# IN2-ViAUn/Exploration-of-Potential

Hardware: AMD Instinct MI355X
Metric: training images/sec, YOLOX-l 24p 640x640 bf16 (higher is better)
Workload: dtype bf16; 1 GPU; YOLOX-l-24p (CSPDarknet53+PAFPN+24p head) train step, 640x640, batch 20/GPU, 10 GTs/img, SimOTA + 24-circle GIoU loss, SGD nesterov; global_batch=20, parallelism=dp1, hip_graph=forward and backward as two lanes of captured segments, loss, update

## Files before the change

exploration-of-potential_amd/csrc/elementwise.hip:

```cpp
#include <stdio.h>
#include <stdlib.h>
#include "common.h"

namespace {

constexpr int MAX_BLOCKS = 2048;

__device__ __forceinline__ void load8(const bf16* p, float (&v)[8]) {
    bf16x8 t = *reinterpret_cast<const bf16x8*>(p);
#pragma unroll
    for (int i = 0; i < 8; ++i) v[i] = (float)t[i];
}
__device__ __forceinline__ void store8(bf16* p, const float (&v)[8]) {
    bf16x8 t;
#pragma unroll
    for (int i = 0; i < 8; ++i) t[i] = (bf16)v[i];
    *reinterpret_cast<bf16x8*>(p) = t;
}

struct RowMap {
    int tpr, rpb;
    __device__ RowMap(int C, int nt = 256) { tpr = C >> 3; rpb = tpr >= nt ? 1 : nt / tpr; }
};

template <int ACT, bool RES>
__global__ __launch_bounds__(256) void bn_act_fwd_kernel(const bf16* z, long ld_z, const long long* stats, int reps,
                                                         const float* gamma, const float* beta, float* rmean,
                                                         float* rvar, long* nbt, long* nbt2, float* save, bf16* y, long ld_y,
                                                         const bf16* res_, long ld_res, long M, int C, float eps,
                                                         float momentum) {
    constexpr int act = ACT;
    const bf16* res = RES ? res_ : nullptr;
    extern __shared__ float lds[];
    const int CP = C + (C >> 3);
    float* sc = lds;
    float* sh = lds + CP;
    auto pad = [](int c) { return c + (c >> 3); };
    for (int c = threadIdx.x; c < C; c += 256) {
        long long i1 = 0, i2 = 0;
        const float gmm = gamma[c], bta = beta[c];
        for (int rb = 0; rb < reps; rb += 8) {
            long long a[8], b[8];
#pragma unroll
            for (int r = 0; r < 8; ++r) {
                const int rr = rb + r < reps ? rb + r : rb;
                a[r] = stats[(long)rr * 2 * C + c];
                b[r] = stats[(long)rr * 2 * C + C + c];
            }
#pragma unroll
            for (int r = 0; r < 8; ++r) {
                i1 += rb + r < reps ? a[r] : 0ll;
                i2 += rb + r < reps ? b[r] : 0ll;
            }
        }
// ... 582 lines not shown
#pragma unroll
                for (int j = 0; j < 8; ++j) {
                    const unsigned byte = ((j < 4 ? c.x : c.y) >> (8 * (j & 3))) & 0xFFu;
                    if ((int)(byte >> 4) == dy + 8) { s[j] += (float)t[j]; sel[j] = (unsigned char)(byte & 15u); }
                }
            }
#pragma unroll
            for (int j = 0; j < 8; ++j) gh[q * 8 + j] = s[j];
            uint2 d;
            d.x = sel[0] | (sel[1] << 8) | (sel[2] << 16) | ((unsigned)sel[3] << 24);
            d.y = sel[4] | (sel[5] << 8) | (sel[6] << 16) | ((unsigned)sel[7] << 24);
            ds[q] = d;
        }
        __syncthreads();
#pragma unroll
        for (int t = 0; t < NPASS; ++t) {
            const int q = threadIdx.x + 256 * t;
            if (q < HW) {
                const int r = q / W, c = q - r * W;
                for (int dxo = -R; dxo <= R; ++dxo) {
                    const int x = c - dxo;
                    if (x < 0 || x >= W) continue;
                    const int o = r * W + x;
                    const uint2 d = ds[o];
#pragma unroll
                    for (int j = 0; j < 8; ++j) {
                        const unsigned byte = ((j < 4 ? d.x : d.y) >> (8 * (j & 3))) & 0xFFu;
                        if ((int)byte == dxo + 8) acc[t][j] += gh[o * 8 + j];
                    }
                }
            }
        }
        __syncthreads();
    }
#pragma unroll
    for (int t = 0; t < NPASS; ++t) {
        const int q = threadIdx.x + 256 * t;
        if (q < HW) {
            bf16* d = dx + (base + q) * ld_dx + cg * 8;
            float out[8];
#pragma unroll
            for (int j = 0; j < 8; ++j) out[j] = acc[t][j];
            if (accumulate) {
                float o[8];
                load8(d, o);
#pragma unroll
                for (int j = 0; j < 8; ++j) out[j] += o[j];
            }
            store8(d, out);
        }
    }
}

__global__ __launch_bounds__(256) void upsample2_fwd_kernel(const bf16* x, long ld_x, bf16* y, long ld_y, int B, int H,
                                                            int W, int C) {
    const int cgs = C >> 3;
    const long total = (long)B * 2 * H * 2 * W * cgs;
    for (long i = (long)blockIdx.x * 256 + threadIdx.x; i < total; i += (long)gridDim.x * 256) {
        const int cg = (int)(i % cgs);
        const long opix = i / cgs;
        const int n = (int)(opix / (4 * H * W));
        const int rem = (int)(opix - (long)n * 4 * H * W);
        const int oy = rem / (2 * W), ox = rem - oy * 2 * W;
        const long ip = (long)(n * H + (oy >> 1)) * W + (ox >> 1);
        *reinterpret_cast<bf16x8*>(y + opix * ld_y + cg * 8) = *reinterpret_cast<const bf16x8*>(x + ip * ld_x + cg * 8);
    }
}

__global__ __launch_bounds__(256) void upsample2_bwd_kernel(const bf16* dy, long ld_dy, bf16* dx, long ld_dx,
                                                            int accumulate, int B, int H, int W, int C) {
    const int cgs = C >> 3;
    const long total = (long)B * H * W * cgs;
    for (long i = (long)blockIdx.x * 256 + threadIdx.x; i < total; i += (long)gridDim.x * 256) {
        const int cg = (int)(i % cgs);
        const long pix = i / cgs;
        const int n = (int)(pix / (H * W));
        const int rem = (int)(pix - (long)n * H * W);
        const int py = rem / W, px = rem - py * W;
        float acc[8] = {0, 0, 0, 0, 0, 0, 0, 0};
#pragma unroll
        for (int a = 0; a < 2; ++a)
#pragma unroll
            for (int b = 0; b < 2; ++b) {
                float v[8];
                load8(dy + ((long)(n * 2 * H + 2 * py + a) * 2 * W + 2 * px + b) * ld_dy + cg * 8, v);
#pragma unroll
                for (int j = 0; j < 8; ++j) acc[j] += v[j];
            }
        bf16* d = dx + pix * ld_dx + cg * 8;
        if (accumulate) {
            float o[8];
            load8(d, o);
#pragma unroll
            for (int j = 0; j < 8; ++j) acc[j] += o[j];
        }
        store8(d, acc);
    }
}

__global__ __launch_bounds__(256) void rows_copy_kernel(const bf16* src, long ld_src, bf16* dst, long ld_dst,
                                                        int accumulate, long M, int C) {
    const int cgs = C >> 3;
    const long total = M * cgs;
    for (long i = (long)blockIdx.x * 256 + threadIdx.x; i < total; i += (long)gridDim.x * 256) {
        const int cg = (int)(i % cgs);
        const long m = i / cgs;
// ... 393 lines not shown
    EP24_REQUIRE(C % 8 == 0 && C <= 2048 && ld_dy % 8 == 0 && ld_z % 8 == 0 && ld_dz % 8 == 0, EP24_E_ARG, "bn_act_bwd_fused: alignment / C <= 2048");
    EP24_REQUIRE((((uintptr_t)save | (uintptr_t)gamma | (uintptr_t)beta | (uintptr_t)gamma_grad | (uintptr_t)beta_grad) & 15) == 0, EP24_E_ARG,
                 "bn_act_bwd_fused: save / gamma / beta and their gradients must be 16-byte aligned (they are read as vectors)");
    int grid = rows_grid(M, C, 4, 256, 256);
    auto kfn = act == 1 ? bn_act_bwd_fused_kernel<1> : act == 2 ? bn_act_bwd_fused_kernel<2> : act == 3 ? bn_act_bwd_fused_kernel<3> : bn_act_bwd_fused_kernel<0>;
    hipLaunchKernelGGL(kfn, dim3(grid), dim3(256), 2 * (size_t)C * sizeof(float), S_, (const bf16*)dy, ld_dy, (const bf16*)z, ld_z, save, gamma, beta,
                       (long long*)dgamma, (long long*)dbeta, gamma_grad, beta_grad, (bf16*)dz, ld_dz, M, C, reps, (unsigned*)barrier);
    EP24_LAUNCH_CHECK("ep24_bn_act_bwd_fused");
    return EP24_OK;
}

namespace ep24_igemm {
int bn_barrier_timeouts() {
    unsigned v = 0;
    if (hipMemcpyFromSymbol(&v, HIP_SYMBOL(g_bn_barrier_timeouts), sizeof(v)) != hipSuccess) return -1;
    return (int)v;
}
}

extern "C" int ep24_bn_act_bwd_apply_acc(const void* dy, int64_t ld_dy, const void* z, int64_t ld_z, const float* save,
                                         const float* gamma, const float* beta, const int64_t* dgamma, const int64_t* dbeta,
                                         float* gamma_grad, float* beta_grad, void* dz, int64_t ld_dz, int64_t M, int C, int act,
                                         int reps, void* stream) {
    EP24_REQUIRE(dy && z && save && gamma && beta && dgamma && dbeta && dz && reps > 0, EP24_E_ARG, "bn_act_bwd_apply_acc: null pointer / reps");
    EP24_REQUIRE(C % 8 == 0 && ld_dy % 8 == 0 && ld_z % 8 == 0 && ld_dz % 8 == 0, EP24_E_ARG, "bn_act_bwd_apply_acc: alignment");
    EP24_REQUIRE((((uintptr_t)save | (uintptr_t)gamma | (uintptr_t)beta) & 15) == 0, EP24_E_ARG,
                 "bn_act_bwd_apply_acc: save / gamma / beta must be 16-byte aligned (they are read as vectors)");
    EP24_REQUIRE((((uintptr_t)gamma_grad | (uintptr_t)beta_grad) & 15) == 0, EP24_E_ARG, "bn_act_bwd_apply_acc: gamma_grad / beta_grad must be 16-byte aligned");
    auto kfn = act == 1 ? bn_act_bwd_apply_kernel<4, 1, true> : act == 2 ? bn_act_bwd_apply_kernel<4, 2, true> : bn_act_bwd_apply_kernel<4, 0, true>;
    hipLaunchKernelGGL(kfn, dim3(rows_grid(M, C, 16, 2048)), dim3(256), 2 * (size_t)C * sizeof(float), S_, (const bf16*)dy, ld_dy, (const bf16*)z, ld_z, save, gamma, beta,
                       (const long long*)dgamma, (const long long*)dbeta, gamma_grad, beta_grad, (bf16*)dz, ld_dz, M, C, reps);
    EP24_LAUNCH_CHECK("ep24_bn_act_bwd_apply_acc");
    return EP24_OK;
}

extern "C" int ep24_stem_pack(const float* images, void* rows, int64_t ld, int B, int H, int W, void* stream) {
    EP24_REQUIRE(images && rows && H % 2 == 0 && W % 2 == 0 && B > 0 && ld >= 108 && ld % 8 == 0, EP24_E_ARG, "stem_pack: bad arguments");
    long sp_blocks = ((long)B * (H / 2) * (W / 2) + 31) / 32;
    hipLaunchKernelGGL(stem_pack_kernel, dim3((unsigned)(sp_blocks > 16384 ? 16384 : sp_blocks)), dim3(256), 0, S_, images,
                       (bf16*)rows, B, H, W, (int)ld);
    EP24_LAUNCH_CHECK("ep24_stem_pack");
    return EP24_OK;
}

extern "C" int ep24_focus_pack(const float* images, void* f16, int B, int H, int W, void* stream) {
    EP24_REQUIRE(images && f16 && H % 2 == 0 && W % 2 == 0 && B > 0 && (reinterpret_cast<unsigned long long>(images) & 7) == 0, EP24_E_ARG,
                 "focus_pack: bad arguments");
    const long blocks = ((long)B * (H / 2) * (W / 2) + 255) / 256;
    hipLaunchKernelGGL(focus_pack_kernel, dim3((unsigned)(blocks > 65536 ? 65536 : blocks)), dim3(256), 0, S_, images, (bf16*)f16, B, H, W);
    EP24_LAUNCH_CHECK("ep24_focus_pack");
    return EP24_OK;
}

extern "C" int ep24_spp_fwd(const void* x, int64_t ld_x, void* y5, void* y9, void* y13, int64_t ld_y, uint8_t* idx, int B,
                            int H, int W, int C, void* scratch, void* stream) {
    EP24_REQUIRE(x && y5 && y9 && y13 && idx && C % 8 == 0 && ld_x % 8 == 0 && ld_y % 8 == 0, EP24_E_ARG, "spp_fwd: bad arguments");
    if (scratch) {
        const long n = (long)B * H * W * C;
        bf16* h = (bf16*)scratch;
        uint8_t* hx = (uint8_t*)scratch + 6 * n;
        hipLaunchKernelGGL(spp_row_kernel, dim3(cap_grid(n / 8)), dim3(256), 0, S_, (const bf16*)x, ld_x, h, hx, B, H, W, C);
        hipLaunchKernelGGL(spp_col_kernel, dim3(cap_grid(n / 8)), dim3(256), 0, S_, (const bf16*)h, (const uint8_t*)hx, (bf16*)y5,
                           (bf16*)y9, (bf16*)y13, ld_y, idx, B, H, W, C);
        EP24_LAUNCH_CHECK("ep24_spp_fwd");
        return EP24_OK;
    }
    hipLaunchKernelGGL(spp_fwd_kernel, dim3(cap_grid((long)B * H * W * (C / 8))), dim3(256), 0, S_, (const bf16*)x, ld_x,
                       (bf16*)y5, (bf16*)y9, (bf16*)y13, ld_y, idx, B, H, W, C);
    EP24_LAUNCH_CHECK("ep24_spp_fwd");
    return EP24_OK;
}

extern "C" int ep24_spp_bwd(const void* dy5, const void* dy9, const void* dy13, int64_t ld_dy, const uint8_t* idx, void* dx,
                            int64_t ld_dx, int accumulate, int B, int H, int W, int C, void* stream) {
    EP24_REQUIRE(dy5 && dy9 && dy13 && idx && dx && C % 8 == 0 && ld_dy % 8 == 0 && ld_dx % 8 == 0, EP24_E_ARG, "spp_bwd: bad arguments");
    const size_t lds = (size_t)H * W * 112;
    if (lds <= 64 * 1024 && H * W <= 1024)
        hipLaunchKernelGGL(spp_bwd_lds_kernel, dim3(C / 8, B), dim3(256), lds, S_, (const bf16*)dy5, (const bf16*)dy9, (const bf16*)dy13,
                           ld_dy, idx, (bf16*)dx, ld_dx, accumulate, B, H, W, C);
    else
        hipLaunchKernelGGL(spp_bwd_kernel, dim3(cap_grid((long)B * H * W * (C / 8))), dim3(256), 0, S_, (const bf16*)dy5,
                           (const bf16*)dy9, (const bf16*)dy13, ld_dy, idx, (bf16*)dx, ld_dx, accumulate, B, H, W, C);
    EP24_LAUNCH_CHECK("ep24_spp_bwd");
    return EP24_OK;
}

extern "C" int ep24_upsample2_fwd(const void* x, int64_t ld_x, void* y, int64_t ld_y, int B, int H, int W, int C, void* stream) {
    EP24_REQUIRE(x && y && C % 8 == 0 && ld_x % 8 == 0 && ld_y % 8 == 0, EP24_E_ARG, "upsample2_fwd: bad arguments");
    hipLaunchKernelGGL(upsample2_fwd_kernel, dim3(cap_grid((long)B * 4 * H * W * (C / 8))), dim3(256), 0, S_, (const bf16*)x,
                       ld_x, (bf16*)y, ld_y, B, H, W, C);
    EP24_LAUNCH_CHECK("ep24_upsample2_fwd");
    return EP24_OK;
}

extern "C" int ep24_upsample2_bwd(const void* dy, int64_t ld_dy, void* dx, int64_t ld_dx, int accumulate, int B, int H, int W,
                                  int C, void* stream) {
    EP24_REQUIRE(dy && dx && C % 8 == 0 && ld_dy % 8 == 0 && ld_dx % 8 == 0, EP24_E_ARG, "upsample2_bwd: bad arguments");
    hipLaunchKernelGGL(upsample2_bwd_kernel, dim3(cap_grid((long)B * H * W * (C / 8))), dim3(256), 0, S_, (const bf16*)dy, ld_dy,
                       (bf16*)dx, ld_dx, accumulate, B, H, W, C);
    EP24_LAUNCH_CHECK("ep24_upsample2_bwd");
    return EP24_OK;
}

extern "C" int ep24_rows_copy(const void* src, int64_t ld_src, void* dst, int64_t ld_dst, int accumulate, int64_t M, int C,
                              void* stream) {
    EP24_REQUIRE(src && dst && C % 8 == 0 && ld_src % 8 == 0 && ld_dst % 8 == 0, EP24_E_ARG, "rows_copy: bad arguments");
    hipLaunchKernelGGL(rows_copy_kernel, dim3(cap_grid(M * (C / 8))), dim3(256), 0, S_, (const bf16*)src, ld_src, (bf16*)dst,
                       ld_dst, accumulate, M, C);
    EP24_LAUNCH_CHECK("ep24_rows_copy");
    return EP24_OK;
}

extern "C" int ep24_cast_f32_bf16(const float* src, void* dst, int64_t n, void* stream) {
    EP24_REQUIRE(src && dst && n % 4 == 0 && n >= 0, EP24_E_ARG, "cast_f32_bf16: n must be a multiple of 4");
    if (n) hipLaunchKernelGGL(cast_f32_bf16_kernel, dim3(cap_grid(n / 4)), dim3(256), 0, S_, src, (bf16*)dst, (long)(n / 4));
    EP24_LAUNCH_CHECK("ep24_cast_f32_bf16");
    return EP24_OK;
}

extern "C" int ep24_cast_bf16_f32(const void* src, float* dst, int64_t n, void* stream) {
    EP24_REQUIRE(src && dst && n % 4 == 0 && n >= 0, EP24_E_ARG, "cast_bf16_f32: n must be a multiple of 4");
    if (n) hipLaunchKernelGGL(cast_bf16_f32_kernel, dim3(cap_grid(n / 4)), dim3(256), 0, S_, (const bf16*)src, dst, (long)(n / 4));
    EP24_LAUNCH_CHECK("ep24_cast_bf16_f32");
    return EP24_OK;
}

extern "C" int ep24_head_decode_fwd(float* out, int B, int A, int a0, int H, int W, float stride, int ncols, float* origin,
                                    void* stream) {
    EP24_REQUIRE(out && a0 >= 0 && a0 + H * W <= A && ncols >= 27, EP24_E_ARG, "head_decode_fwd: bad arguments");
    hipLaunchKernelGGL(decode_fwd_kernel, dim3(cap_grid((long)B * H * W * 26)), dim3(256), 0, S_, out, B, A, a0, H, W, stride, ncols, origin);
    EP24_LAUNCH_CHECK("ep24_head_decode_fwd");
    return EP24_OK;
}

extern "C" int ep24_head_decode_bwd(const float* dout, const float* out, void* d_regobj, void* d_cls, int B, int A, int a0,
                                    int H, int W, float stride, int ncols, const float* d_origin, void* stream) {
    EP24_REQUIRE(dout && out && d_regobj && d_cls && a0 >= 0 && a0 + H * W <= A && ncols > 27, EP24_E_ARG,
// ... 145 lines not shown
```

exploration-of-potential_amd/ep24/engine.py:

```python
import torch

from . import _lib, nn as enn
from ._lib import call, ptr, stream_ptr
from .options import PlanOptions, get_options

BF16 = torch.bfloat16
WGRAD_REDUCE_GROUP = 16
WGRAD_GROUP_MAX = 16
WGRAD_GROUP_FILL = 0.88
WGRAD_GROUP_TAIL = 0.93
STATS_REPLICAS = 8
STRIDES = (8, 16, 32)


def _r8(n):
    return (n + 7) // 8 * 8


class Buf:

    def __init__(self, dev, rows, ld, dtype=BF16):
        self.rows, self.ld, self.dtype = rows, ld, dtype
        self.esize = 4 if dtype == torch.float32 else 2
        self.t = torch.zeros(rows * ld, dtype=dtype, device=dev)
# ... 499 lines not shown
            raise IndexError("ep24: empty input size %s" % (size,))
        self.model, self.B, self.S = model, batch, self.IH
        self.dtype, self.f32 = dtype, dtype == torch.float32
        self.home = param_home(model)
        self.dev = self.home.dev
        self.C = getattr(getattr(model, "head", None), "num_classes", 0)
        self.ncols = 27 + self.C
        self.fwd, self.bwd = [], []
        self.outputs = None
        self.unit_acts = {}
        self.fwd_eval = []
        self.bwd_writes = []
        self.bwd_gw, self.bwd_rd = [], []
        self._bwd_units = 0
        self._cur_tag = None
        self._force_side = False
        self._deferred = []
        self.bwd_tail_cut = None
        self.bwd_join = None
        self.bwd_par_end = None
        self.options = model.__dict__.get("_ep24_options") or getattr(self.home, "options", None) or get_options(model)
        if self.options.layout() != self.home.options.layout():
            raise _lib.Ep24Error("ep24: this model's parameters are laid out for %r; the merge options cannot change afterwards" % (self.home.options,))
        self.parallel_head = self.options.parallel_head and not self.f32
        self._dz_elems = 0
        self._slab_floats, self._pending_reduce, self._keep = 0, [], []
        self.head_grads = []
        self.skip_decode_bwd = False
        self._wg_pending = {}
        self._wg_tail = False
        self._side = None
        self.use_side = not self.f32
        self.capture_side = self.options.capture_side
        self._events = []
        self._bwd_builders = []
        self.pre_bn_inputs = {}
        self.fold_bn_eval = self.options.fold_bn_eval
        self._fold_units, self._fold_w, self._fold_c = [], 0, 0
        self.dyn = {"origin": None, "d_origin": None}
        self.origin = None
        self._stats_specs, self._sum_specs = [], []
        self.max_dz = 0
        self._build()

    def new_act(self, C, H, W, ld=None):
        return Act(Buf(self.dev, self.B * H * W, ld or C, self.dtype), 0, C, self.B, H, W)

    def _kopt(self, name, args):
        ko = self.options.conv_kernel_opts
        if ko & 0xFF and name in ("conv_fwd_bf16", "conv_dgrad_bf16"):
            return name + "_ex", tuple(args) + (ko & 0xFF,)
        if ko & 0x100 and name in ("conv_wgrad_slab_bf16", "side:conv_wgrad_slab_bf16"):
            return name + "_ex", tuple(args) + (1,)
        return name, tuple(args)

    def _wsplits(self, B, H, W, cin, cout, k, s):
        return _lib.lib().fn["ep24_conv_wgrad_splits_ex"](B, H, W, cin, cout, k, s, 1 if self.options.conv_kernel_opts & 0x100 else 0)

    def _f(self, name, *args, ev=None):
        name, args = self._kopt(name, args)
        self.fwd.append((name, args))
        if ev is not False:
            self.fwd_eval.append(ev if ev is not None else (name, args))

    def _b(self, name, args, writes=(), reads=None):
        name, args = self._kopt(name, args)
        if self._force_side and name[0] != "@" and not name.startswith("side:"):
            name = "side:" + name
        self.bwd.append((name, args))
        self.bwd_writes.append([(seg.off, seg.numel) for seg in writes])
        self.bwd_gw.append(list(_PENDING_GW))
        del _PENDING_GW[:]
        self.bwd_rd.append(reads.gregion() if reads is not None else None)

    def _build(self):
        m, B = self.model, self.B
        bb, neck, head = m.backbone.backbone, m.backbone, m.head
        if self.IH % 32 or self.IW % 32:
            raise IndexError("ep24: the input height and width must be multiples of 32 (three stride levels), got %dx%d" % (self.IH, self.IW))
        self.images = torch.zeros(B, 3, self.IH, self.IW, dtype=torch.float32, device=self.dev)
        x2, x1, x0 = self.build_neck_inputs(neck)
        pans = self.build_neck(neck, x2, x1, x0)
        self.build_head(head, pans)
        self._finalize()

    def neck_channels(self, bb):
        swapped = isinstance(bb, (enn.ResNet, enn.DenseNet, enn.VGG))
        if swapped and self.f32:
            raise NotImplementedError("ep24: the fp32 parity mode covers the CSPDarknet network (the BASELINE configuration)")
        return (256, 512, 1024) if swapped else tuple(_units(st[0])[-1].conv.out_channels for st in (bb.dark3, bb.dark4, bb.dark5))

    def focus_stem(self, focus):
        B = self.B
        if self.f32:
            rows = self.new_act(112, self.IH // 2, self.IW // 2)
            rows.needs_grad = False
            self._f("f32_stem_pack", ptr(self.images), rows.ptr(), 112, B, self.IH, self.IW)
            return self.unit(focus.conv, rows, stem=True)
        f16 = self.new_act(16, self.IH // 2, self.IW // 2)
        f16.needs_grad = False
        self._f("focus_pack", ptr(self.images), f16.ptr(), B, self.IH, self.IW)
        return self.unit(focus.conv, f16, stem="focus")

    def build_backbone(self, bb, out3=None, out4=None):
        B = self.B
        if isinstance(bb, (enn.ResNet, enn.DenseNet, enn.VGG)):
# ... 674 lines not shown
        c3 = self.unit(None, feats[1], out=out3, conv=bb.baseconv1.conv, bn=bb.baseconv1.bn, act=2)
        c4 = self.unit(None, feats[2], out=out4, conv=bb.baseconv2.conv, bn=bb.baseconv2.bn, act=2)
        return c3, c4, feats[3]

    def avgpool2(self, x, y):
        self._f("avgpool2_fwd", x.ptr(), x.ld, y.ptr(), y.ld, x.B, x.H, x.W, x.C)

        def build_bwd():
            assert y.gready()
            acc = x.gwrite()
            self._b("avgpool2_bwd", (y.gptr(), y.gld, x.gptr(), x.gld, acc, x.B, x.H, x.W, x.C))

        self._add_builder(build_bwd)
        return y

    def draw_dropout(self):
        if getattr(self, "drop_keep", None) is not None and not getattr(self, "fixed_dropout", False):
            self.drop_keep.bernoulli_(1.0 - self.drop_p).div_(1.0 - self.drop_p)

    def csp_merged(self, mod, x, out=None):
        h = mod.conv1.conv.out_channels
        _same_bn(mod.conv2.bn, mod.conv1.bn)
        P = self.new_act(3 * h, x.H, x.W)
        both = P.slice(h, 2 * h)
        self.unit(None, x, out=both, conv=mod.conv2.conv, bn=mod.conv2.bn, act=mod.conv2.act_code, bn2=mod.conv1.bn)
        xa, za, ya = self.unit_acts.pop(mod.conv2.conv)
        self.unit_acts[mod.conv2] = (xa, za.slice(0, h), ya.slice(0, h))
        self.unit_acts[mod.conv1] = (xa, za.slice(h, h), ya.slice(h, h))
        t = x1 = P.slice(2 * h, h)
        n = len(mod.m)
        if any(blk.use_add for blk in mod.m):
            raw = P.slice(2 * h, h)

            def build_copy():
                assert x1._alias is not None and x1._groot().buf.gwritten
                acc = raw.gwrite()
                self._b("f32_rows_copy" if self.f32 else "rows_copy", (x1.gptr(), x1.gld, raw.gptr(), raw.gld, acc, x1.M, h))

            self._add_builder(build_copy)
        for i, blk in enumerate(mod.m):
            u = self.unit(blk.conv1, t, bn_in=i > 0, below_in=i > 0)
            t = self.conv_block(blk.conv2, u, out=P.slice(0, h) if i == n - 1 else None, residual=t if blk.use_add else None, x_single=True)
        return self.unit(mod.conv3, P.slice(0, 2 * h), out=out)

    def spp(self, mod, x):
        h = self.home.by_param[mod.conv1.conv.weight].cout
        cat = self.new_act(4 * h, x.H, x.W)
        t = self.unit(mod.conv1, x, out=cat.slice(0, h))
        y5, y9, y13 = cat.slice(h, h), cat.slice(2 * h, h), cat.slice(3 * h, h)
        idx = torch.zeros(3 * t.M * h, dtype=torch.int32 if self.f32 else torch.uint8, device=self.dev)
        if self.f32:
            self._f("f32_spp_fwd", t.ptr(), t.ld, y5.ptr(), y9.ptr(), y13.ptr(), cat.ld, ptr(idx), t.B, t.H, t.W, h, ev=False)
        else:
            scratch = torch.zeros(9 * t.M * h, dtype=torch.uint8, device=self.dev)
            self._keep.append(scratch)
            self._f("spp_fwd", t.ptr(), t.ld, y5.ptr(), y9.ptr(), y13.ptr(), cat.ld, ptr(idx), t.B, t.H, t.W, h, ptr(scratch))

        def build_bwd():
            assert y5.gready() and y9.gready() and y13.gready()
            acc = t.gwrite()
            self._b("f32_spp_bwd" if self.f32 else "spp_bwd", (y5.gptr(), y9.gptr(), y13.gptr(), y5.gld, ptr(idx), t.gptr(), t.gld, acc,
                                                                t.B, t.H, t.W, h))

        self._add_builder(build_bwd)
        return self.unit(mod.conv2, cat)

    def up2(self, x, y):
        pre = "f32_" if self.f32 else ""
        self._f(pre + "upsample2_fwd", x.ptr(), x.ld, y.ptr(), y.ld, x.B, x.H, x.W, x.C, ev=False if self.f32 else None)

        def build_bwd():
            assert y.gready()
            acc = x.gwrite()
            self._b(pre + "upsample2_bwd", (y.gptr(), y.gld, x.gptr(), x.gld, acc, x.B, x.H, x.W, x.C))

        self._add_builder(build_bwd)

    def head_level(self, head, k, feat, a0):
        home, B, C = self.home, self.B, self.C
        H, W, s = feat.H, feat.W, float(head.strides[k])
        self.levels.append((H, W, s))
        self._cur_tag = ("head", k)
        x = self.unit(head.stems[k], feat)
        if head_is_merged(head, self.options):
            c0, r0 = head.cls_convs[k][0], head.reg_convs[k][0]
            hc = c0.conv.out_channels
            _same_bn(c0.bn, r0.bn)
            both = self.unit(None, x, conv=c0.conv, bn=c0.bn, act=c0.act_code, bn2=r0.bn, x_single=True)
            xa, za, ya = self.unit_acts.pop(c0.conv)
            self.unit_acts[c0] = (xa, za.slice(0, hc), ya.slice(0, hc))
            self.unit_acts[r0] = (xa, za.slice(hc, hc), ya.slice(hc, hc))
            cf = self.unit(head.cls_convs[k][1], both.slice(0, hc), x_single=True)
            rf = self.unit(head.reg_convs[k][1], both.slice(hc, hc), x_single=True)
        else:
            cf = self.conv_block(head.cls_convs[k][1], self.conv_block(head.cls_convs[k][0], x), x_single=True)
            rf = self.conv_block(head.reg_convs[k][1], self.conv_block(head.reg_convs[k][0], x), x_single=True)
        ro_seg = home.by_param[head.reg_preds[k].weight]
        ro_b = home.by_param[head.reg_preds[k].bias]
        cl_seg = home.by_param[head.cls_preds[k].weight]
        cl_b = home.by_param[head.cls_preds[k].bias]
        hch = x.C
        M = B * H * W
        out = self.outputs
        flat, gflat = home.flat, home.gflat
        if self.f32:
            return self._head_preds_f32(rf, cf, ro_seg, ro_b, cl_seg, cl_b, hch, M, a0, H, W, s)
        self._f("conv_fwd_bf16", rf.ptr(), rf.ld, ptr(home.wf, ro_seg.wf_off), ptr(out), self.ncols, 1, self.A, a0,
                ptr(flat, ro_b.off), None, 1, B, H, W, hch, 27, 1, 1)
# ... 388 lines not shown
```

exploration-of-potential_amd/ep24/options.py:

```python
from dataclasses import dataclass, fields, replace
from typing import ClassVar, Optional, Tuple


@dataclass(frozen=True)
class PlanOptions:
    merge_csp: bool = True
    merge_csp_shortcut: bool = True
    merge_head: bool = True
    parallel_head: bool = True
    capture_side: bool = False
    fold_bn_eval: bool = True
    conv_kernel_opts: int = 0
    wgrad_group_steps: int = 100
    group_wgrad: bool = True
    fuse_bn_reduce: bool = False
    fuse_bn_bwd: bool = False
    fuse_bn_stream: bool = True
    fuse_bn_dgrad: bool = True
    fuse_bn_reduce_stream: bool = True
    fuse_loss_decode: bool = True
    parallel_forward: bool = True
    forward_lanes: int = 2
    head1_side: bool = True
    cost_on_lanes: bool = True
    tail_cuts: bool = True
    bwd_cuts: Optional[Tuple[float, ...]] = None
    chunked_update: bool = True

    LAYOUT_FIELDS: ClassVar[tuple] = ("merge_csp", "merge_csp_shortcut", "merge_head")

    def with_(self, **kw):
        return replace(self, **kw)

    def layout(self):
        return tuple(getattr(self, k) for k in self.LAYOUT_FIELDS)

    @classmethod
    def parse(cls, text):
        kw = {}
        types = {f.name: f.type for f in fields(cls)}
        for item in filter(None, (text or "").split(",")):
            k, _, v = item.partition("=")
            k = k.strip()
            if k not in types:
                raise ValueError("unknown plan option %r (known: %s)" % (k, ", ".join(sorted(types))))
            if k == "bwd_cuts":
                kw[k] = (tuple((i + 1) / int(v[1:]) for i in range(int(v[1:]) - 1)) if v[0] == "u"
                         else tuple(float(x) for x in v.split(":")))
            elif k in ("forward_lanes", "conv_kernel_opts", "wgrad_group_steps"):
                kw[k] = int(v)
            else:
                kw[k] = v.strip() not in ("0", "false", "False", "")
        return cls(**kw)


DEFAULT = PlanOptions()


def set_options(model, options):
    home = model.__dict__.get("_ep24_home")
    if home is not None and home.options.layout() != options.layout():
        from ._lib import Ep24Error
        raise Ep24Error("ep24: the merge options must be set before the model first runs (its parameters already live in flat "
                        "buffers laid out for %r)" % (home.options,))
    model.__dict__["_ep24_options"] = options
    return model


def get_options(model):
    return model.__dict__.get("_ep24_options", DEFAULT)
```

include/ep24.h:

```cpp
#ifndef EP24_H
#define EP24_H
#include <stdint.h>

#ifdef __cplusplus
extern "C" {
#endif

#define EP24_OK 0
#define EP24_E_ARG (-1)
#define EP24_E_LAUNCH (-2)
#define EP24_E_UNSUPPORTED (-3)

#define EP24_MAX_GT 50
#define EP24_RAYS 24
#define EP24_LABEL_COLS 51
#define EP24_NUM_SUMS 32

const char* ep24_last_error(void);
#define EP24_ABI_VERSION 3
int ep24_abi_version(void);


int ep24_conv_fwd_bf16(const void* x, int64_t ld_x, const void* w, void* y, int64_t ld_y, int y_f32,
                       int64_t y_batch_rows, int64_t y_row0, const float* bias, int64_t* stats, int stats_replicas,
// ... 69 lines not shown
int ep24_dwconv_wgrad_slab_bf16(const void* x, int64_t ld_x, const void* dz, int64_t ld_dz, float* slab, int64_t slab_floats, int B,
                                int H, int W, int C, int ksize, int stride, void* stream);

int ep24_conv1x1_xf_ok(int B, int H, int W, int Cin, int Cout);
int ep24_conv1x1_bnin_bf16(const void* z_in, int64_t ld_zin, const int64_t* stats_in, int reps_in, const float* gamma,
                           const float* beta, float* running_mean, float* running_var, int64_t* num_batches,
                           int64_t* num_batches2, float* save, void* y_in, int64_t ld_yin, const void* residual, int64_t ld_res,
                           float eps, float momentum, int act, const void* w, void* z_out, int64_t ld_zout, int64_t* stats_out,
                           int reps_out, int B, int H, int W, int Cin, int Cout, void* stream);
int ep24_conv1x1_dgrad_bnbwd_bf16(const void* dy, int64_t ld_dy, const void* z, int64_t ld_z, const float* save,
                                  const float* gamma, const float* beta, const int64_t* dgamma, const int64_t* dbeta,
                                  float* gamma_grad, float* beta_grad, void* dz, int64_t ld_dz, int act, int reps, const void* wt,
                                  void* dx, int64_t ld_dx, int accumulate, int B, int H, int W, int Cin, int Cout_k, void* stream);

int ep24_f32_stem_pack(const float* images, float* rows, int64_t ld, int B, int H, int W, void* stream);
int ep24_f32_conv(const float* x, int64_t ld_x, const float* w, int64_t w_co_stride, int64_t w_tap_stride, float* y, int64_t ld_y,
                  int64_t y_batch_rows, int64_t y_row0, const float* bias, int accumulate, int B, int H, int W, int Cin, int Cout,
                  int ksize, int stride, int transposed, void* stream);
int ep24_f32_conv_wgrad(const float* x, int64_t ld_x, const float* dy, int64_t ld_dy, float* dw, int64_t w_co_stride,
                        int64_t w_tap_stride, int B, int H, int W, int Cin, int Cout, int ksize, int stride, void* stream);
int ep24_f32_bn_act_fwd(const float* z, int64_t ld_z, const float* gamma, const float* beta, float* running_mean, float* running_var,
                        int64_t* num_batches, float* save, float* y, int64_t ld_y, const float* residual, int64_t ld_res, int64_t M,
                        int C, float eps, float momentum, int act, void* stream);
int ep24_f32_bn_act_bwd(const float* dy, int64_t ld_dy, const float* z, int64_t ld_z, const float* save, const float* gamma,
                        const float* beta, double* sums, float* gamma_grad, float* beta_grad, float* dz, int64_t ld_dz, int64_t M,
                        int C, int act, void* stream);
int ep24_f32_spp_fwd(const float* x, int64_t ld_x, float* y5, float* y9, float* y13, int64_t ld_y, int32_t* idx, int B, int H, int W,
                     int C, void* stream);
int ep24_f32_spp_bwd(const float* dy5, const float* dy9, const float* dy13, int64_t ld_dy, const int32_t* idx, float* dx,
                     int64_t ld_dx, int accumulate, int B, int H, int W, int C, void* stream);
int ep24_f32_upsample2_fwd(const float* x, int64_t ld_x, float* y, int64_t ld_y, int B, int H, int W, int C, void* stream);
int ep24_f32_upsample2_bwd(const float* dy, int64_t ld_dy, float* dx, int64_t ld_dx, int accumulate, int B, int H, int W, int C,
                           void* stream);
int ep24_f32_rows_copy(const float* src, int64_t ld_src, float* dst, int64_t ld_dst, int accumulate, int64_t M, int C, void* stream);
int ep24_f32_head_decode_bwd(const float* dout, const float* out, float* d_regobj, float* d_cls, int B, int A, int a0, int H, int W,
                             float stride, int ncols, const float* d_origin, void* stream);
int ep24_f32_colsum(const float* g, int64_t ld, float* db, int64_t M, int N, void* stream);

int ep24_stem_pack(const float* images, void* rows, int64_t ld, int B, int H, int W, void* stream);

int ep24_focus_pack(const float* images, void* f16, int B, int H, int W, void* stream);
int ep24_stem_conv_fwd_bf16(const void* f16, const void* w, int64_t ld_w, void* y, int64_t ld_y, int64_t* stats, int stats_replicas,
                            int B, int FH, int FW, int Cout, void* stream);
int ep24_stem_conv_fwd_infer_bf16(const void* f16, const void* w, int64_t ld_w, const float* bias, int act, void* y, int64_t ld_y,
                                  int B, int FH, int FW, int Cout, void* stream);
int ep24_stem_conv_wgrad_slab_bf16(const void* f16, const void* dy, int64_t ld_dy, float* slab, int64_t slab_floats, int B, int FH,
                                   int FW, int Cout, void* stream);
int ep24_stem_conv_wgrad_splits(int B, int FH, int FW, int Cout);

int ep24_spp_fwd(const void* x, int64_t ld_x, void* y5, void* y9, void* y13, int64_t ld_y, uint8_t* idx,
                 int B, int H, int W, int C, void* scratch, void* stream);
int ep24_spp_bwd(const void* dy5, const void* dy9, const void* dy13, int64_t ld_dy, const uint8_t* idx,
                 void* dx, int64_t ld_dx, int accumulate, int B, int H, int W, int C, void* stream);

int ep24_upsample2_fwd(const void* x, int64_t ld_x, void* y, int64_t ld_y, int B, int H, int W, int C, void* stream);
int ep24_upsample2_bwd(const void* dy, int64_t ld_dy, void* dx, int64_t ld_dx, int accumulate,
                       int B, int H, int W, int C, void* stream);

int ep24_memset_zero(void* p, int64_t bytes, void* stream);
int ep24_cast_f32_bf16(const float* src, void* dst, int64_t n, void* stream);
int ep24_cast_bf16_f32(const void* src, float* dst, int64_t n, void* stream);

int ep24_rows_copy(const void* src, int64_t ld_src, void* dst, int64_t ld_dst, int accumulate, int64_t M, int C,
                   void* stream);

int ep24_head_decode_fwd(float* out, int B, int A, int a0, int H, int W, float stride, int ncols, float* origin,
                         void* stream);
int ep24_head_decode_bwd(const float* dout, const float* out, void* d_regobj, void* d_cls, int B, int A, int a0,
                         int H, int W, float stride, int ncols, const float* d_origin, void* stream);
int ep24_colsum(const void* g, int64_t ld, float* db, int64_t M, int N, void* stream);
int ep24_colsum_splits(int64_t M);
int ep24_colsum_slab(const void* g, int64_t ld, float* slab, int64_t M, int N, void* stream);

int ep24_assign_candidates(const float* labels, const float* xs, const float* ys, const float* strides,
                           int32_t* num_gt, uint64_t* in_box, uint64_t* in_ctr, int B, int A, void* stream);
int ep24_assign_cost(const float* outputs, int ncols, const float* labels, const int32_t* num_gt,
                     const uint64_t* in_box, const uint64_t* in_ctr, float* pw, float* cost, int B, int A,
                     int num_classes, void* stream);
int ep24_assign_cost_range(const float* outputs, int ncols, const float* labels, const int32_t* num_gt,
                           const uint64_t* in_box, const uint64_t* in_ctr, float* pw, float* cost, int B, int A,
                           int num_classes, int a_lo, int a_hi, void* stream);
int ep24_dynamic_k(const float* pw, const float* cost, const int32_t* num_gt, const uint64_t* in_box,
                   const uint64_t* in_ctr, uint64_t* match, int32_t* ks, int B, int A, void* stream);
int ep24_assign_resolve(const uint64_t* match, const float* pw, const float* cost, const int32_t* num_gt,
                        int32_t* matched_gt, float* matched_iou, int B, int A, void* stream);

int ep24_loss_blocks(int B, int A);
int ep24_loss_terms(const float* outputs, int ncols, const float* labels, const int32_t* matched_gt,
                    const float* matched_iou, float* partials, int B, int A, int num_classes, const float* origin,
                    const float* xs, const float* ys, const float* strides, void* stream);
int ep24_loss_finalize(const float* partials, int nblocks, const int32_t* num_gt, int B, float* state, float* result,
                       void* stream);
int ep24_loss_grad(const float* outputs, int ncols, const float* labels, const int32_t* matched_gt,
                   const float* matched_iou, const float* result, const float* grad_scale, float* dout, int B, int A,
                   int num_classes, const float* origin, const float* xs, const float* ys, const float* strides,
                   float* d_origin, void* stream);

int ep24_loss_grad_decode(const float* outputs, int ncols, const float* labels, const int32_t* matched_gt, const float* matched_iou,
                          const float* result, int B, int A, int num_classes, int n_levels, const int64_t* levels, void* stream);

int ep24_circle_pairwise(const float* gt50, const float* pred26, float* out, int G, int P, void* stream);
int ep24_circle_matched_fwd(const float* pred26, const float* target50, float* loss24, int N, void* stream);
int ep24_circle_matched_bwd(const float* pred26, const float* target50, const float* dloss24, float* dpred26, int N,
                            void* stream);
int ep24_circle_lens(const float* gt_cx, const float* gt_cy, const float* gt_r, const float* pd_cx, const float* pd_cy,
                     const float* pd_r, float* res_inter, float* dist, int G, int P, int pairwise, void* stream);
// ... 114 lines not shown
```

Before: 1041 images/s.

## Add LDS-tiled channel-slice SPP forward and backward kernels

Adds SPP max-pool forward and backward kernels that stage one image's channel slice in LDS. Each kernel computes the separable 5/9/13 row and column passes there, so the global scratch buffer and its extra kernel launch go away. The scratch allocation is now made only when the legacy path is forced. Blocks are interleaved across groups of eight, and dynamic LDS up to 128 KB is opted into per device. The SPP layer is small at 20x20 resolution, so the effect on the whole training step is limited. The new path also depends on LDS capacity and on occupancy.

Result: no change. 1045 images/s, median of 6 (+0.4%).

```diff
diff --git a/exploration-of-potential_amd/csrc/elementwise.hip b/exploration-of-potential_amd/csrc/elementwise.hip
--- a/exploration-of-potential_amd/csrc/elementwise.hip
+++ b/exploration-of-potential_amd/csrc/elementwise.hip
@@ -1,5 +1,6 @@
 #include <stdio.h>
 #include <stdlib.h>
+#include <atomic>
 #include "common.h"
 
 namespace {
@@ -688,6 +689,206 @@
     }
 }
 
+__device__ __forceinline__ bool spp_slice_of_block(int B, int C, int CS, int& n, int& c0, int& g) {
+    const int slices = (C + CS - 1) / CS;
+    const int nblk = B * slices, per = (nblk + 7) >> 3;
+    const int l = (int)(blockIdx.x & 7) * per + (int)(blockIdx.x >> 3);
+    if (l >= nblk) return false;
+    n = l / slices;
+    c0 = (l - n * slices) * CS;
+    g = ((C - c0 < CS) ? C - c0 : CS) >> 3;
+    return true;
+}
+
+__device__ __forceinline__ uint2 pack8(const unsigned (&c)[8]) {
+    uint2 d;
+    d.x = c[0] | (c[1] << 8) | (c[2] << 16) | (c[3] << 24);
+    d.y = c[4] | (c[5] << 8) | (c[6] << 16) | (c[7] << 24);
+    return d;
+}
+
+template <int R>
+__device__ __forceinline__ void spp_lds_rows(const bf16* xs, bf16* hs, uint2* hx, int items, int g, int W) {
+    for (int it = threadIdx.x; it < items; it += 256) {
+        const int px = (it / g) % W;
+        float m[8];
+        unsigned c[8];
+#pragma unroll
+        for (int j = 0; j < 8; ++j) { m[j] = -INFINITY; c[j] = 8u; }
+#pragma unroll
+        for (int dx = -R; dx <= R; ++dx) {
+            const int xx = px + dx;
+            if (xx < 0 || xx >= W) continue;
+            float v[8];
+            load8(xs + (long)(it + dx * g) * 8, v);
+#pragma unroll
+            for (int j = 0; j < 8; ++j)
+                if (v[j] > m[j] || v[j] != v[j]) { m[j] = v[j]; c[j] = (unsigned)(dx + 8); }
+        }
+        store8(hs + (long)it * 8, m);
+        hx[it] = pack8(c);
+    }
+}
+
+template <int R>
+__device__ __forceinline__ void spp_lds_cols(const bf16* hs, const uint2* hx, bf16* y, long ld_y, uint8_t* codes, long base, int C,
+                                             int c0, int items, int g, int H, int W) {
+    for (int it = threadIdx.x; it < items; it += 256) {
+        const int q = it / g, k = it - q * g;
+        const int py = q / W;
+        float m[8];
+        unsigned c[8];
+#pragma unroll
+        for (int j = 0; j < 8; ++j) { m[j] = -INFINITY; c[j] = 0x88u; }
+#pragma unroll
+        for (int dy = -R; dy <= R; ++dy) {
+            const int yy = py + dy;
+            if (yy < 0 || yy >= H) continue;
+            const int o = it + dy * W * g;
+            float v[8];
+            load8(hs + (long)o * 8, v);
+            const uint2 cx = hx[o];
+#pragma unroll
+            for (int j = 0; j < 8; ++j) {
+                const unsigned b = ((j < 4 ? cx.x : cx.y) >> (8 * (j & 3))) & 0xFFu;
+                if (v[j] > m[j] || v[j] != v[j]) { m[j] = v[j]; c[j] = (unsigned)((dy + 8) << 4) | b; }
+            }
+        }
+        store8(y + (base + q) * ld_y + c0 + k * 8, m);
+        *reinterpret_cast<uint2*>(codes + (base + q) * C + c0 + k * 8) = pack8(c);
+    }
+}
+
+__global__ __launch_bounds__(256) void spp_fwd_lds_kernel(const bf16* x, long ld_x, bf16* y5, bf16* y9, bf16* y13, long ld_y,
+                                                          uint8_t* idx, int B, int H, int W, int C, int CS) {
+    extern __shared__ __attribute__((aligned(16))) char spp_lds[];
+    int n, c0, g;
+    if (!spp_slice_of_block(B, C, CS, n, c0, g)) return;
+    const int HW = H * W;
+    const int items = HW * g;
+    bf16* xs = reinterpret_cast<bf16*>(spp_lds);
+    bf16* hs = xs + (size_t)HW * CS;
+    uint2* hx = reinterpret_cast<uint2*>(spp_lds + (size_t)HW * CS * 4);
+    const long base = (long)n * HW;
+    const long plane = (long)B * HW * C;
+    for (int it = threadIdx.x; it < items; it += 256) {
+        const int q = it / g, k = it - q * g;
+        *reinterpret_cast<bf16x8*>(xs + (long)it * 8) = *reinterpret_cast<const bf16x8*>(x + (base + q) * ld_x + c0 + k * 8);
+    }
+    __syncthreads();
+    spp_lds_rows<2>(xs, hs, hx, items, g, W);
+    __syncthreads();
+    spp_lds_cols<2>(hs, hx, y5, ld_y, idx, base, C, c0, items, g, H, W);
+    __syncthreads();
+    spp_lds_rows<4>(xs, hs, hx, items, g, W);
+    __syncthreads();
+    spp_lds_cols<4>(hs, hx, y9, ld_y, idx + plane, base, C, c0, items, g, H, W);
+    __syncthreads();
+    spp_lds_rows<6>(xs, hs, hx, items, g, W);
+    __syncthreads();
+    spp_lds_cols<6>(hs, hx, y13, ld_y, idx + 2 * plane, base, C, c0, items, g, H, W);
+}
+
+template <int NPASS>
+__global__ __launch_bounds__(256) void spp_bwd_slice_kernel(const bf16* dy5, const bf16* dy9, const bf16* dy13, long ld_dy,
+                                                            const uint8_t* idx, bf16* dx, long ld_dx, int accumulate, int B,
+                                                            int H, int W, int C, int CS) {
+    extern __shared__ __attribute__((aligned(16))) char spp_lds[];
+    int n, c0, g;
+    if (!spp_slice_of_block(B, C, CS, n, c0, g)) return;
+    const int HW = H * W;
+    const int items = HW * g;
+    float* gh = reinterpret_cast<float*>(spp_lds);
+    bf16x8* gs = reinterpret_cast<bf16x8*>(spp_lds + (size_t)HW * CS * 4);
+    uint2* cs = reinterpret_cast<uint2*>(spp_lds + (size_t)HW * CS * 6);
+    uint2* ds = reinterpret_cast<uint2*>(spp_lds + (size_t)HW * CS * 7);
+    const long base = (long)n * HW;
+    const long plane = (long)B * HW * C;
+    float acc[NPASS][8];
+#pragma unroll
+    for (int t = 0; t < NPASS; ++t)
+#pragma unroll
+        for (int j = 0; j < 8; ++j) acc[t][j] = 0.f;
+    for (int pool = 2; pool >= 0; --pool) {
+        const int R = 2 * pool + 2;
+        const bf16* gy = pool == 2 ? dy13 : (pool == 1 ? dy9 : dy5);
+        const uint8_t* codes = idx + pool * plane;
+        for (int it = threadIdx.x; it < items; it += 256) {
+            const int q = it / g, k = it - q * g;
+            gs[it] = *reinterpret_cast<const bf16x8*>(gy + (base + q) * ld_dy + c0 + k * 8);
+            cs[it] = *reinterpret_cast<const uint2*>(codes + (base + q) * C + c0 + k * 8);
+        }
+        __syncthreads();
+        for (int it = threadIdx.x; it < items; it += 256) {
+            const int r = (it / g) / W;
+            float s[8] = {0, 0, 0, 0, 0, 0, 0, 0};
+            unsigned sel[8];
+#pragma unroll
+            for (int j = 0; j < 8; ++j) sel[j] = 0xFFu;
+            for (int dy = -R; dy <= R; ++dy) {
+                const int y = r - dy;
+                if (y < 0 || y >= H) continue;
+                const int o = it - dy * W * g;
+                const uint2 c = cs[o];
+                const bf16x8 t = gs[o];
+                const unsigned want = (unsigned)(dy + 8);
+#pragma unroll
+                for (int j = 0; j < 8; ++j) {
+                    const unsigned byte = ((j < 4 ? c.x : c.y) >> (8 * (j & 3))) & 0xFFu;
+                    const bool hit = (byte >> 4) == want;
+                    s[j] += hit ? (float)t[j] : 0.f;
+                    sel[j] = hit ? (byte & 15u) : sel[j];
+                }
+            }
+            float4* o4 = reinterpret_cast<float4*>(gh + (long)it * 8);
+            o4[0] = make_float4(s[0], s[1], s[2], s[3]);
+            o4[1] = make_float4(s[4], s[5], s[6], s[7]);
+            ds[it] = pack8(sel);
+        }
+        __syncthreads();
+#pragma unroll
+        for (int t = 0; t < NPASS; ++t) {
+            const int it = threadIdx.x + 256 * t;
+            if (it < items) {
+                const int c = (it / g) % W;
+                for (int dxo = -R; dxo <= R; ++dxo) {
+                    const int x = c - dxo;
+                    if (x < 0 || x >= W) continue;
+                    const int o = it - dxo * g;
+                    const uint2 d = ds[o];
+                    const float4* s4 = reinterpret_cast<const float4*>(gh + (long)o * 8);
+                    const float4 lo = s4[0], hi = s4[1];
+                    const float s[8] = {lo.x, lo.y, lo.z, lo.w, hi.x, hi.y, hi.z, hi.w};
+                    const unsigned want = (unsigned)(dxo + 8);
+#pragma unroll
+                    for (int j = 0; j < 8; ++j) {
+                        const unsigned byte = ((j < 4 ? d.x : d.y) >> (8 * (j & 3))) & 0xFFu;
+                        acc[t][j] += byte == want ? s[j] : 0.f;
+                    }
+                }
+            }
+        }
+    }
+#pragma unroll
+    for (int t = 0; t < NPASS; ++t) {
+        const int it = threadIdx.x + 256 * t;
+        if (it < items) {
+            const int q = it / g, k = it - q * g;
+            bf16* d = dx + (base + q) * ld_dx + c0 + k * 8;
+            float out[8];
+#pragma unroll
+            for (int j = 0; j < 8; ++j) out[j] = acc[t][j];
+            if (accumulate) {
+                float o[8];
+                load8(d, o);
+#pragma unroll
+                for (int j = 0; j < 8; ++j) out[j] += o[j];
+            }
+            store8(d, out);
+        }
+    }
+}
+
 __global__ __launch_bounds__(256) void upsample2_fwd_kernel(const bf16* x, long ld_x, bf16* y, long ld_y, int B, int H,
                                                             int W, int C) {
     const int cgs = C >> 3;
@@ -1187,9 +1388,53 @@
     return EP24_OK;
 }
 
-extern "C" int ep24_spp_fwd(const void* x, int64_t ld_x, void* y5, void* y9, void* y13, int64_t ld_y, uint8_t* idx, int B,
-                            int H, int W, int C, void* scratch, void* stream) {
-    EP24_REQUIRE(x && y5 && y9 && y13 && idx && C % 8 == 0 && ld_x % 8 == 0 && ld_y % 8 == 0, EP24_E_ARG, "spp_fwd: bad arguments");
+namespace {
+
+constexpr size_t SPP_LDS_TWO = 80 * 1024, SPP_LDS_MAX = 128 * 1024;
+constexpr int SPP_MAX_PIXELS = 2048;
+int spp_slice_width(int B, int HW, int C, int bpe, int forced) {
+    if (HW > SPP_MAX_PIXELS) return 0;
+    if (forced) return (forced % 8 == 0 && (size_t)HW * forced * bpe <= SPP_LDS_MAX) ? forced : 0;
+    int cs = 8;
+    while (cs < 64 && cs * 2 <= C && (size_t)HW * cs * 2 * bpe <= SPP_LDS_TWO) cs *= 2;
+    while (cs > 16 && (long)B * ((C + cs - 1) / cs) < 512) cs /= 2;
+    return cs;
+}
+
+template <typename K>
+int spp_lds_optin(K kernel, std::atomic<unsigned long long>& done) {
+    int dev = 0;
+    EP24_REQUIRE(hipGetDevice(&dev) == hipSuccess, EP24_E_LAUNCH, "spp: hipGetDevice failed");
+    const unsigned long long bit = 1ull << (dev & 63);
+    if (!(done.load(std::memory_order_acquire) & bit)) {
+        const hipError_t e = hipFuncSetAttribute((const void*)kernel, hipFuncAttributeMaxDynamicSharedMemorySize, (int)SPP_LDS_MAX);
+        EP24_REQUIRE(e == hipSuccess, EP24_E_LAUNCH, "spp: hipFuncSetAttribute(MaxDynamicSharedMemorySize, %d) failed on device %d: %s",
+                     (int)SPP_LDS_MAX, dev, hipGetErrorString(e));
+        done.fetch_or(bit, std::memory_order_release);
+    }
+    return EP24_OK;
+}
+
+}
+
+extern "C" int ep24_spp_fwd_ex(const void* x, int64_t ld_x, void* y5, void* y9, void* y13, int64_t ld_y, uint8_t* idx, int B,
+                               int H, int W, int C, void* scratch, int opts, void* stream) {
+    EP24_REQUIRE(x && y5 && y9 && y13 && idx && C % 8 == 0 && ld_x % 8 == 0 && ld_y % 8 == 0 && B > 0 && H > 0 && W > 0 && C > 0 &&
+                     !(opts & ~0xFF01),
+                 EP24_E_ARG, "spp_fwd: bad arguments");
+    const int cs = (opts & 1) || (reinterpret_cast<unsigned long long>(idx) & 7) || (long)H * W > SPP_MAX_PIXELS
+                       ? 0 : spp_slice_width(B, H * W, C, 5, (opts >> 8) & 0xFF);
+    EP24_REQUIRE(cs || !(opts >> 8), EP24_E_ARG, "spp_fwd: the forced slice width does not fit");
+    if (cs) {
+        static std::atomic<unsigned long long> done{0};
+        const int rc = spp_lds_optin(spp_fwd_lds_kernel, done);
+        if (rc != EP24_OK) return rc;
+        const int nblk = B * ((C + cs - 1) / cs);
+        hipLaunchKernelGGL(spp_fwd_lds_kernel, dim3(8 * ((nblk + 7) / 8)), dim3(256), (size_t)H * W * cs * 5, S_, (const bf16*)x, ld_x,
+                           (bf16*)y5, (bf16*)y9, (bf16*)y13, ld_y, idx, B, H, W, C, cs);
+        EP24_LAUNCH_CHECK("ep24_spp_fwd");
+        return EP24_OK;
+    }
     if (scratch) {
         const long n = (long)B * H * W * C;
         bf16* h = (bf16*)scratch;
@@ -1206,9 +1451,31 @@
     return EP24_OK;
 }
 
-extern "C" int ep24_spp_bwd(const void* dy5, const void* dy9, const void* dy13, int64_t ld_dy, const uint8_t* idx, void* dx,
-                            int64_t ld_dx, int accumulate, int B, int H, int W, int C, void* stream) {
-    EP24_REQUIRE(dy5 && dy9 && dy13 && idx && dx && C % 8 == 0 && ld_dy % 8 == 0 && ld_dx % 8 == 0, EP24_E_ARG, "spp_bwd: bad arguments");
+extern "C" int ep24_spp_fwd(const void* x, int64_t ld_x, void* y5, void* y9, void* y13, int64_t ld_y, uint8_t* idx, int B,
+                            int H, int W, int C, void* scratch, void* stream) {
+    return ep24_spp_fwd_ex(x, ld_x, y5, y9, y13, ld_y, idx, B, H, W, C, scratch, 0, stream);
+}
+
+extern "C" int ep24_spp_bwd_ex(const void* dy5, const void* dy9, const void* dy13, int64_t ld_dy, const uint8_t* idx, void* dx,
+                               int64_t ld_dx, int accumulate, int B, int H, int W, int C, int opts, void* stream) {
+    EP24_REQUIRE(dy5 && dy9 && dy13 && idx && dx && C % 8 == 0 && ld_dy % 8 == 0 && ld_dx % 8 == 0 && B > 0 && H > 0 && W > 0 && C > 0 &&
+                     !(opts & ~0xFF01),
+                 EP24_E_ARG, "spp_bwd: bad arguments");
+    const int cs = (opts & 1) || (reinterpret_cast<unsigned long long>(idx) & 7) || (long)H * W > SPP_MAX_PIXELS
+                       ? 0 : spp_slice_width(B, H * W, C, 8, (opts >> 8) & 0xFF);
+    EP24_REQUIRE(cs || !(opts >> 8), EP24_E_ARG, "spp_bwd: the forced slice width does not fit");
+    if (cs) {
+        static std::atomic<unsigned long long> done4{0}, done8{0};
+        const bool wide = (long)H * W * (cs / 8) > 256 * 4;
+        const int rc = wide ? spp_lds_optin(spp_bwd_slice_kernel<8>, done8) : spp_lds_optin(spp_bwd_slice_kernel<4>, done4);
+        if (rc != EP24_OK) return rc;
+        const int nblk = B * ((C + cs - 1) / cs);
+        hipLaunchKernelGGL(wide ? spp_bwd_slice_kernel<8> : spp_bwd_slice_kernel<4>, dim3(8 * ((nblk + 7) / 8)), dim3(256),
+                           (size_t)H * W * cs * 8, S_, (const bf16*)dy5, (const bf16*)dy9, (const bf16*)dy13, ld_dy, idx, (bf16*)dx, ld_dx,
+                           accumulate, B, H, W, C, cs);
+        EP24_LAUNCH_CHECK("ep24_spp_bwd");
+        return EP24_OK;
+    }
     const size_t lds = (size_t)H * W * 112;
     if (lds <= 64 * 1024 && H * W <= 1024)
         hipLaunchKernelGGL(spp_bwd_lds_kernel, dim3(C / 8, B), dim3(256), lds, S_, (const bf16*)dy5, (const bf16*)dy9, (const bf16*)dy13,
@@ -1218,6 +1485,11 @@
                            (const bf16*)dy9, (const bf16*)dy13, ld_dy, idx, (bf16*)dx, ld_dx, accumulate, B, H, W, C);
     EP24_LAUNCH_CHECK("ep24_spp_bwd");
     return EP24_OK;
+}
+
+extern "C" int ep24_spp_bwd(const void* dy5, const void* dy9, const void* dy13, int64_t ld_dy, const uint8_t* idx, void* dx,
+                            int64_t ld_dx, int accumulate, int B, int H, int W, int C, void* stream) {
+    return ep24_spp_bwd_ex(dy5, dy9, dy13, ld_dy, idx, dx, ld_dx, accumulate, B, H, W, C, 0, stream);
 }
 
 extern "C" int ep24_upsample2_fwd(const void* x, int64_t ld_x, void* y, int64_t ld_y, int B, int H, int W, int C, void* stream) {
diff --git a/exploration-of-potential_amd/ep24/engine.py b/exploration-of-potential_amd/ep24/engine.py
--- a/exploration-of-potential_amd/ep24/engine.py
+++ b/exploration-of-potential_amd/ep24/engine.py
@@ -575,6 +575,8 @@
             return name + "_ex", tuple(args) + (ko & 0xFF,)
         if ko & 0x100 and name in ("conv_wgrad_slab_bf16", "side:conv_wgrad_slab_bf16"):
             return name + "_ex", tuple(args) + (1,)
+        if self.options.spp_kernel_opts and name in ("spp_fwd", "spp_bwd"):
+            return name + "_ex", tuple(args) + (self.options.spp_kernel_opts,)
         return name, tuple(args)
 
     def _wsplits(self, B, H, W, cin, cout, k, s):
@@ -1355,8 +1357,10 @@
         if self.f32:
             self._f("f32_spp_fwd", t.ptr(), t.ld, y5.ptr(), y9.ptr(), y13.ptr(), cat.ld, ptr(idx), t.B, t.H, t.W, h, ev=False)
         else:
-            scratch = torch.zeros(9 * t.M * h, dtype=torch.uint8, device=self.dev)
-            self._keep.append(scratch)
+            scratch = None
+            if self.options.spp_kernel_opts & 1:
+                scratch = torch.zeros(9 * t.M * h, dtype=torch.uint8, device=self.dev)
+                self._keep.append(scratch)
             self._f("spp_fwd", t.ptr(), t.ld, y5.ptr(), y9.ptr(), y13.ptr(), cat.ld, ptr(idx), t.B, t.H, t.W, h, ptr(scratch))
 
         def build_bwd():
diff --git a/exploration-of-potential_amd/ep24/options.py b/exploration-of-potential_amd/ep24/options.py
--- a/exploration-of-potential_amd/ep24/options.py
+++ b/exploration-of-potential_amd/ep24/options.py
@@ -11,6 +11,7 @@
     capture_side: bool = False
     fold_bn_eval: bool = True
     conv_kernel_opts: int = 0
+    spp_kernel_opts: int = 0
     wgrad_group_steps: int = 100
     group_wgrad: bool = True
     fuse_bn_reduce: bool = False
@@ -47,7 +48,7 @@
             if k == "bwd_cuts":
                 kw[k] = (tuple((i + 1) / int(v[1:]) for i in range(int(v[1:]) - 1)) if v[0] == "u"
                          else tuple(float(x) for x in v.split(":")))
-            elif k in ("forward_lanes", "conv_kernel_opts", "wgrad_group_steps"):
+            elif k in ("forward_lanes", "conv_kernel_opts", "spp_kernel_opts", "wgrad_group_steps"):
                 kw[k] = int(v)
             else:
                 kw[k] = v.strip() not in ("0", "false", "False", "")
diff --git a/include/ep24.h b/include/ep24.h
--- a/include/ep24.h
+++ b/include/ep24.h
@@ -145,6 +145,10 @@
                  int B, int H, int W, int C, void* scratch, void* stream);
 int ep24_spp_bwd(const void* dy5, const void* dy9, const void* dy13, int64_t ld_dy, const uint8_t* idx,
                  void* dx, int64_t ld_dx, int accumulate, int B, int H, int W, int C, void* stream);
+int ep24_spp_fwd_ex(const void* x, int64_t ld_x, void* y5, void* y9, void* y13, int64_t ld_y, uint8_t* idx,
+                    int B, int H, int W, int C, void* scratch, int opts, void* stream);
+int ep24_spp_bwd_ex(const void* dy5, const void* dy9, const void* dy13, int64_t ld_dy, const uint8_t* idx,
+                    void* dx, int64_t ld_dx, int accumulate, int B, int H, int W, int C, int opts, void* stream);
 
 int ep24_upsample2_fwd(const void* x, int64_t ld_x, void* y, int64_t ld_y, int B, int H, int W, int C, void* stream);
 int ep24_upsample2_bwd(const void* dy, int64_t ld_dy, void* dx, int64_t ld_dx, int accumulate,
```
